# ORNL/HydraGNN

Measured on NVIDIA H100. Metric: atoms_per_sec_training_step, higher is better.
Workload: dtype tf32

## Files before the change

hydragnn_b200/csrc/hgb_painn.cu:

```cuda
#include "hgb_common.cuh"

#define RMAX 8
#define WPB 8

template <int G>
__device__ __forceinline__ float hgb_group_sum(float v, unsigned mask) {
#pragma unroll
  for (int o = G / 2; o > 0; o >>= 1) v += __shfl_xor_sync(mask, v, o);
  return v;
}

#define EPK 12

template <int CPL>
struct ChanVec;
template <>
struct ChanVec<1> {
  static __device__ __forceinline__ void ld(const float* p, float* o) { o[0] = __ldg(p); }
  static __device__ __forceinline__ void st(float* p, const float* o) { p[0] = o[0]; }
};
template <>
struct ChanVec<2> {
  static __device__ __forceinline__ void ld(const float* p, float* o) { const float2 t = __ldg(reinterpret_cast<const float2*>(p)); o[0] = t.x; o[1] = t.y; }
  static __device__ __forceinline__ void st(float* p, const float* o) { *reinterpret_cast<float2*>(p) = make_float2(o[0], o[1]); }
// ... 127 lines not shown
               : "memory");
}

#define TWPB 10
__device__ __forceinline__ float2 pm_lds_f2(uint32_t addr) {
  float2 r;
  asm volatile("ld.shared.v2.f32 {%0, %1}, [%2];" : "=f"(r.x), "=f"(r.y) : "r"(addr));
  return r;
}
__device__ __forceinline__ void pm_cp_async16(void* smem, const void* g) {
  asm volatile("cp.async.ca.shared.global [%0], [%1], 16;" ::"r"((uint32_t)__cvta_generic_to_shared(smem)), "l"(g) : "memory");
}
__device__ __forceinline__ void pm_cp_async_commit() { asm volatile("cp.async.commit_group;" ::: "memory"); }
__device__ __forceinline__ void pm_cp_async_wait_all() { asm volatile("cp.async.wait_group 0;" ::: "memory"); }

template <bool HAS_EF, int RT, int FT>
__global__ void __launch_bounds__(TWPB * 32, 2)
painn_message_fwd_tiled_kernel(const float* __restrict__ phi, const float* __restrict__ s, const float* __restrict__ v,
                               const int32_t* __restrict__ rowptr, const float* __restrict__ rec, const float* __restrict__ wf,
                               const float* __restrict__ bf, const float* __restrict__ efilt, int n, int f_rt, int r, int tn,
                               float* __restrict__ s_out, float* __restrict__ v_out) {
  extern __shared__ __align__(128) uint8_t pm_smem[];
  const int f = FT ? FT : f_rt;
  const int f3 = 3 * f;
  const uint32_t tile_bytes = (uint32_t)tn * f3 * 4;
  auto sphi = [&](int b) { return reinterpret_cast<float*>(pm_smem + (size_t)(2 * b) * tile_bytes); };
  auto sv = [&](int b) { return reinterpret_cast<float*>(pm_smem + (size_t)(2 * b + 1) * tile_bytes); };
  uint64_t* full = reinterpret_cast<uint64_t*>(pm_smem + 4 * (size_t)tile_bytes);
  uint64_t* empty = full + 2;
  float4* scr = reinterpret_cast<float4*>(full + 4) + (threadIdx.x >> 5) * 96;
  const int lane = threadIdx.x & 31, warp = threadIdx.x >> 5;
  const int ntiles = (n + tn - 1) / tn;
  const int ncb = f >> 6;
  if (threadIdx.x == 0) {
    pm_mbar_init(full, 1);
    pm_mbar_init(full + 1, 1);
    pm_mbar_init(empty, TWPB);
    pm_mbar_init(empty + 1, TWPB);
    asm volatile("fence.mbarrier_init.release.cluster;" ::: "memory");
  }
  __syncthreads();
  auto issue = [&](int t, int buf) {
    const int n0 = t * tn;
    const uint32_t bytes = (uint32_t)(min(n, n0 + tn) - n0) * f3 * 4;
    pm_mbar_expect_tx(full + buf, 2 * bytes);
    pm_bulk_g2s(sphi(buf), phi + (int64_t)n0 * f3, bytes, full + buf);
    pm_bulk_g2s(sv(buf), v + (int64_t)n0 * f3, bytes, full + buf);
  };
  if (threadIdx.x == 0 && (int)blockIdx.x < ntiles) issue(blockIdx.x, 0);
  const float4* rec4 = reinterpret_cast<const float4*>(rec);
  auto succ = [&](int i, int& tile, int& cb) {
    int in = i + TWPB;
    if (in < min(n, tile * tn + tn)) return in;
    if (++cb == ncb) { cb = 0; tile += (int)gridDim.x; }
    in = tile * tn + warp;
    return (tile < ntiles && in < min(n, tile * tn + tn)) ? in : -1;
  };
  auto stage = [&](int in, int cbn, int lo_n, int hi_n, float4* dst) {
    if (lane < 4 * min(8, hi_n - lo_n)) pm_cp_async16(dst + lane, rec4 + (int64_t)lo_n * 4 + lane);
// ... 13 lines not shown
  int it = 0;
  for (int t = blockIdx.x; t < ntiles; t += gridDim.x, ++it) {
    const int buf = it & 1;
    const int tnext = t + gridDim.x;
    if (warp == 0 && tnext < ntiles) {
      if (it >= 1) pm_mbar_wait(empty + (buf ^ 1), ((it - 1) >> 1) & 1);
      if (lane == 0) issue(tnext, buf ^ 1);
      __syncwarp();
    }
    pm_mbar_wait(full + buf, (it >> 1) & 1);
    const int n0 = t * tn, n1 = min(n, n0 + tn);
    const float* tv = sv(buf);
    const uint32_t tphi_u = pm_smem_u32(sphi(buf)), tv_u = pm_smem_u32(sv(buf));
    for (int cb = 0; cb < ncb; ++cb) {
      const int cc = cb * 64 + lane * 2;
      float wr[3][2][RT + 1];
#pragma unroll
      for (int a = 0; a < 3; ++a)
#pragma unroll
        for (int tt = 0; tt < 2; ++tt) {
#pragma unroll
          for (int q = 0; q < RT; ++q) wr[a][tt][q] = q < r ? __ldg(wf + (a * f + cc + tt) * r + q) : 0.f;
          wr[a][tt][RT] = __ldg(bf + a * f + cc + tt);
        }
      for (int i = n0 + warp; i < n1; i += TWPB) {
        pm_cp_async_wait_all();
        __syncwarp();
        const float4* cur = scr + sb * 48;
        int inn = -1, lo_nn = 0, hi_nn = 0;
        if (in >= 0) {
// ... 10 lines not shown
            e0 = ep[0]; e1 = ep[1]; e2 = ep[2]; e3 = ep[3];
          } else {
            const float4* ep = rec4 + (int64_t)p * 4;
            e0 = __ldg(ep); e1 = __ldg(ep + 1); e2 = __ldg(ep + 2); e3 = __ldg(ep + 3);
          }
          const float rb[8] = {e0.x, e0.y, e0.z, e0.w, e1.x, e1.y, e1.z, e1.w};
          const float fce = e2.x, d[3] = {e2.y, e2.z, e2.w};
          const int j = __float_as_int(e3.x);
          const int e = __float_as_int(e3.y);
          (void)e;
          float pv[3][2], vv[3][2];
          if (j >= n0 && j < n1) {
            const uint32_t off = (uint32_t)((j - n0) * f3 + cc) * 4u;
#pragma unroll
            for (int a = 0; a < 3; ++a) {
              const float2 x2 = pm_lds_f2(tphi_u + off + a * f * 4), y2 = pm_lds_f2(tv_u + off + a * f * 4);
              pv[a][0] = x2.x; pv[a][1] = x2.y; vv[a][0] = y2.x; vv[a][1] = y2.y;
            }
          } else {
            const float* ph = phi + (int64_t)j * f3 + cc;
            const float* vj = v + (int64_t)j * f3 + cc;
#pragma unroll
            for (int a = 0; a < 3; ++a) { ChanVec<2>::ld(ph + a * f, pv[a]); ChanVec<2>::ld(vj + a * f, vv[a]); }
          }
          float ef[3][2];
          if (HAS_EF) {
#pragma unroll
            for (int a = 0; a < 3; ++a) ChanVec<2>::ld(efilt + (int64_t)e * f3 + a * f + cc, ef[a]);
          }
#pragma unroll
          for (int tt = 0; tt < 2; ++tt) {
            float w[3];
#pragma unroll
            for (int a = 0; a < 3; ++a) {
              float acc = wr[a][tt][RT] * fce;
#pragma unroll
              for (int q = 0; q < RT; ++q) acc = fmaf(wr[a][tt][q], rb[q], acc);
              w[a] = HAS_EF ? acc * ef[a][tt] : acc;
            }
            const float gv = w[0] * pv[0][tt], ge = w[1] * pv[1][tt];
            as[tt] = fmaf(w[2], pv[2][tt], as[tt]);
#pragma unroll
            for (int k = 0; k < 3; ++k) av[k][tt] = fmaf(ge, d[k], fmaf(vv[k][tt], gv, av[k][tt]));
          }
        }
        const float2 own_s = *(reinterpret_cast<const float2*>(cur + 32) + lane);
        float so[2] = {own_s.x + as[0], own_s.y + as[1]}, tmp[2];
        ChanVec<2>::st(s_out + (int64_t)i * f + cc, so);
#pragma unroll
        for (int k = 0; k < 3; ++k) {
          const float2 own = *reinterpret_cast<const float2*>(tv + (size_t)(i - n0) * f3 + k * f + cc);
          tmp[0] = own.x + av[k][0]; tmp[1] = own.y + av[k][1];
          ChanVec<2>::st(v_out + (int64_t)i * f3 + k * f + cc, tmp);
        }
        lo = lo_n; hi = hi_n; sb ^= 1;
        in = inn; lo_n = lo_nn; hi_n = hi_nn;
      }
    }
    __syncwarp();
    if (lane == 0) pm_mbar_arrive(empty + buf);
  }
}

static int painn_group(int f) { int g = 32; if (f < 32) { g = 1; while (g < f) g <<= 1; } return g; }
static int painn_cpl(int f) { return (f >= 64 && f % 2 == 0) ? 2 : 1; }

extern "C" int hgb_painn_message_fwd(const float* phi, const float* s, const float* v, const int32_t* rowptr,
                                     const int32_t* perm, const int32_t* nbr, const float* epack, const float* rec, const float* wf,
                                     const float* bf, const float* efilt, int32_t n, int32_t f, int32_t r, float* s_out, float* v_out,
                                     hgb_stream_t stream) {
  HGB_REQUIRE(n >= 0 && f > 0 && r > 0 && r <= RMAX, "painn_message_fwd: need 0 < num_radial <= %d (got %d)", RMAX, r);
  HGB_REQUIRE(phi && s && v && rowptr && nbr && epack && wf && bf && s_out && v_out, "painn_message_fwd: null pointer");
  if (n == 0) return HGB_OK;
  cudaStream_t st = (cudaStream_t)stream;
  if (rec && f % 64 == 0 && f <= 256 && n >= 256 && (((uintptr_t)phi | (uintptr_t)v | (uintptr_t)s | (uintptr_t)rec) % 16 == 0)) {
    int tn = (int)((110 * 1024 - TWPB * 1536 - 64) / ((size_t)4 * 3 * f * 4));
    tn = (tn / TWPB) * TWPB;
    if (tn > 3 * TWPB) tn = 3 * TWPB;
    if (tn < TWPB) tn = TWPB;
    const size_t smem = (size_t)4 * tn * 3 * f * 4 + 64 + TWPB * 1536;
    static bool attr_done = false;
    if (!attr_done) {
#define SETA(E, R) cudaFuncSetAttribute(painn_message_fwd_tiled_kernel<E, R, 64>, cudaFuncAttributeMaxDynamicSharedMemorySize, 227 * 1024); \
                   cudaFuncSetAttribute(painn_message_fwd_tiled_kernel<E, R, 0>, cudaFuncAttributeMaxDynamicSharedMemorySize, 227 * 1024)
      SETA(false, 5); SETA(false, 8); SETA(true, 5); SETA(true, 8);
#undef SETA
      attr_done = true;
    }
    const int ntiles = (n + tn - 1) / tn;
    const int g1 = ntiles < 2 * HGB_NUM_SMS ? ntiles : 2 * HGB_NUM_SMS;
#define LAUNCH_F(E, R, F) painn_message_fwd_tiled_kernel<E, R, F><<<g1, TWPB * 32, smem, st>>>(phi, s, v, rowptr, rec, wf, bf, efilt, n, f, r, tn, s_out, v_out)
#define LAUNCH_T(E, R) do { if (f == 64) LAUNCH_F(E, R, 64); else LAUNCH_F(E, R, 0); } while (0)
    if (efilt) { if (r <= 5) LAUNCH_T(true, 5); else LAUNCH_T(true, 8); }
    else { if (r <= 5) LAUNCH_T(false, 5); else LAUNCH_T(false, 8); }
#undef LAUNCH_T
#undef LAUNCH_F
    HGB_LAUNCH_CHECK("painn_message_fwd_tiled");
    return HGB_OK;
  }
  const int cpl = painn_cpl(f), group = painn_group(f);
  dim3 grid(hgb_grid_for(n, WPB * (32 / group), HGB_NUM_SMS * 8), (f + group * cpl - 1) / (group * cpl));
#define LAUNCH(C, E, G, R) painn_message_fwd_kernel<C, E, G, R><<<grid, WPB * 32, 0, st>>>(phi, s, v, rowptr, perm, nbr, epack, wf, bf, efilt, n, f, r, s_out, v_out)
#define LAUNCH_R(C, E, G) do { if (r <= 5) LAUNCH(C, E, G, 5); else LAUNCH(C, E, G, 8); } while (0)
#define LAUNCH_G(E)                                                        \
  switch (group) {                                                         \
    case 1: LAUNCH_R(1, E, 1); break;                                      \
    case 2: LAUNCH_R(1, E, 2); break;                                      \
// ... 153 lines not shown
          __syncthreads();
          red[warp * 32 + lane] = gw[a][t][q];
          __syncthreads();
          if (warp == 0 && lane < GROUP) {
            float acc = 0.f;
#pragma unroll
            for (int w8 = 0; w8 < WPB; ++w8)
#pragma unroll
              for (int g = 0; g < NPW; ++g) acc += red[w8 * 32 + lane + GROUP * g];
            if (ok) mypart[(a * f + cc + t) * (r + 1) + (q == RT ? r : q)] = acc;
          }
        }
      }
}

template <bool HAS_EF, bool NEED_EDGE, int RT, int FT>
__global__ void __launch_bounds__(WPB * 32, 2)
painn_message_bwd_tiled_kernel(const float* __restrict__ gs_out, const float* __restrict__ gv_out, const float* __restrict__ phi,
                               const float* __restrict__ v, const int32_t* __restrict__ rowptr, const float* __restrict__ rec,
                               const float* __restrict__ wf, const float* __restrict__ bf, const float* __restrict__ efilt, int n,
                               int f_rt, int r, int tn, float* __restrict__ gphi, float* __restrict__ gv, float* __restrict__ part,
                               float* __restrict__ g_epack, float* __restrict__ g_efilt, int multi_cb) {
  extern __shared__ __align__(128) uint8_t pm_smem[];
  const int f = FT ? FT : f_rt;
  const int f3 = 3 * f;
  const uint32_t gs_bytes = (uint32_t)tn * f * 4, gv_bytes = (uint32_t)tn * f3 * 4;
  auto sgs = [&](int b) { return reinterpret_cast<float*>(pm_smem + (size_t)b * (gs_bytes + gv_bytes)); };
  auto sgv = [&](int b) { return reinterpret_cast<float*>(pm_smem + (size_t)b * (gs_bytes + gv_bytes) + gs_bytes); };
  uint64_t* full = reinterpret_cast<uint64_t*>(pm_smem + 2 * ((size_t)gs_bytes + gv_bytes));
  uint64_t* empty = full + 2;
  float* red = reinterpret_cast<float*>(full + 4);
  float4* scr = reinterpret_cast<float4*>(red + WPB * 32) + (threadIdx.x >> 5) * 256;
  const int lane = threadIdx.x & 31, warp = threadIdx.x >> 5;
  const int ntiles = (n + tn - 1) / tn;
  if (threadIdx.x == 0) {
    pm_mbar_init(full, 1);
    pm_mbar_init(full + 1, 1);
// ... 14 lines not shown
  const int cc = cb * 64 + lane * 2;
  float wr[3][2][RT + 1], gw[3][2][RT + 1];
#pragma unroll
  for (int a = 0; a < 3; ++a)
#pragma unroll
    for (int t = 0; t < 2; ++t) {
#pragma unroll
      for (int q = 0; q < RT; ++q) { wr[a][t][q] = q < r ? wf[(a * f + cc + t) * r + q] : 0.f; gw[a][t][q] = 0.f; }
      wr[a][t][RT] = bf[a * f + cc + t];
      gw[a][t][RT] = 0.f;
    }
  const float4* rec4 = reinterpret_cast<const float4*>(rec);
  auto stage = [&](int jn, int lo_n, int hi_n, float4* dst) {
    if (lane < 4 * min(8, hi_n - lo_n)) pm_cp_async16(dst + lane, rec4 + (int64_t)lo_n * 4 + lane);
    const float* pj = phi + (int64_t)jn * f3 + cb * 64;
    const float* vjp = v + (int64_t)jn * f3 + cb * 64;
    pm_cp_async16(dst + 32 + lane, pj + (lane >> 4) * f + (lane & 15) * 4);
    pm_cp_async16(dst + 80 + lane, vjp + (lane >> 4) * f + (lane & 15) * 4);
    if (lane < 16) {
      pm_cp_async16(dst + 64 + lane, pj + 2 * f + lane * 4);
      pm_cp_async16(dst + 112 + lane, vjp + 2 * f + lane * 4);
    }
  };
  auto succ = [&](int j, int& tile) {
    int jn = j + WPB;
    if (jn < min(n, tile * tn + tn)) return jn;
    tile += (int)gridDim.x;
    jn = tile * tn + warp;
    return (tile < ntiles && jn < min(n, tile * tn + tn)) ? jn : -1;
  };
  int lo = 0, hi = 0, sb = 0, lo_n = 0, hi_n = 0, jn = -1, tile_n = blockIdx.x;
  {
    const int j0 = blockIdx.x * tn + warp;
    if ((int)blockIdx.x < ntiles && j0 < min(n, (int)blockIdx.x * tn + tn)) {
      lo = rowptr[j0]; hi = rowptr[j0 + 1];
      stage(j0, lo, hi, scr);
// ... 15 lines not shown
    const int n0 = tile * tn, n1 = min(n, n0 + tn);
    const float* tgv = sgv(buf);
    const uint32_t tgs_u = pm_smem_u32(sgs(buf)), tgv_u = pm_smem_u32(sgv(buf));
    for (int j = n0 + warp; j < n1; j += WPB) {
      pm_cp_async_wait_all();
      __syncwarp();
      const float4* cur = scr + sb * 128;
      int jnn = -1, lo_nn = 0, hi_nn = 0;
      if (jn >= 0) {
        stage(jn, lo_n, hi_n, scr + (sb ^ 1) * 128);
        jnn = succ(jn, tile_n);
        if (jnn >= 0) { lo_nn = rowptr[jnn]; hi_nn = rowptr[jnn + 1]; }
      }
      pm_cp_async_commit();
      float ph[3][2], vj[3][2], aphi[3][2], agv[3][2];
#pragma unroll
      for (int a = 0; a < 3; ++a) {
        const float2 p2 = *(reinterpret_cast<const float2*>(cur + 32 + a * 16) + lane);
        const float2 v2 = *(reinterpret_cast<const float2*>(cur + 80 + a * 16) + lane);
        ph[a][0] = p2.x; ph[a][1] = p2.y; vj[a][0] = v2.x; vj[a][1] = v2.y;
        aphi[a][0] = aphi[a][1] = 0.f; agv[a][0] = agv[a][1] = 0.f;
      }
      for (int p = lo; p < hi; ++p) {
        float4 e0, e1, e2, e3;
        if (p - lo < 8) {
          const float4* ep = cur + (p - lo) * 4;
          e0 = ep[0]; e1 = ep[1]; e2 = ep[2]; e3 = ep[3];
        } else {
          const float4* ep = rec4 + (int64_t)p * 4;
          e0 = __ldg(ep); e1 = __ldg(ep + 1); e2 = __ldg(ep + 2); e3 = __ldg(ep + 3);
        }
        const float rb[8] = {e0.x, e0.y, e0.z, e0.w, e1.x, e1.y, e1.z, e1.w};
        const float fce = e2.x, d[3] = {e2.y, e2.z, e2.w};
        const int i = __float_as_int(e3.x);
        const int e = __float_as_int(e3.y);
// ... 137 lines not shown
  if (threadIdx.y == 0 && t < cnt) {
    float sum = 0.f;
#pragma unroll
    for (int w8 = 0; w8 < 8; ++w8) sum += red[w8][threadIdx.x];
    const int row = t / (r + 1), q = t % (r + 1);
    if (q == r) gbf[row] = sum; else gwf[row * r + q] = sum;
  }
}

static int painn_bwd_grid(int n, int f) { return hgb_grid_for(n, WPB * (32 / painn_group(f)), HGB_NUM_SMS * (f < 32 ? 2 : 4)); }

extern "C" int64_t hgb_painn_message_bwd_workspace_bytes(int32_t n, int32_t f, int32_t r) {
  return (int64_t)painn_bwd_grid(n, f) * 3 * f * (r + 1) * 4;
}

extern "C" int hgb_painn_message_bwd(const float* gs_out, const float* gv_out, const float* phi, const float* v,
                                     const int32_t* rowptr_src, const int32_t* perm_src, const int32_t* nbr_agg, const float* epack,
                                     const float* rec, const float* wf, const float* bf, const float* efilt, int32_t n, int32_t f, int32_t r,
                                     float* gphi, float* gv, float* gwf, float* gbf, float* g_epack, float* g_efilt, void* workspace,
                                     int64_t workspace_bytes, hgb_stream_t stream) {
  HGB_REQUIRE(n >= 0 && f > 0 && r > 0 && r <= RMAX, "painn_message_bwd: need 0 < num_radial <= %d (got %d)", RMAX, r);
  HGB_REQUIRE(gs_out && gv_out && phi && v && rowptr_src && nbr_agg && epack && wf && bf && gphi && gv && gwf && gbf && workspace,
              "painn_message_bwd: null pointer");
  const bool need_edge = g_epack != nullptr;
  HGB_REQUIRE((efilt != nullptr) == (g_efilt != nullptr), "painn_message_bwd: g_efilt iff efilt");
  HGB_REQUIRE(workspace_bytes >= hgb_painn_message_bwd_workspace_bytes(n, f, r), "painn_message_bwd: workspace too small");
  cudaStream_t st = (cudaStream_t)stream;
  const int f3 = 3 * f;
  if (n == 0) {
    cudaMemsetAsync(gwf, 0, (size_t)f3 * r * 4, st);
    cudaMemsetAsync(gbf, 0, (size_t)f3 * 4, st);
    return HGB_OK;
  }
  float* part = (float*)workspace;
  if (rec && f % 64 == 0 && f <= 256 && n >= 256 && (((uintptr_t)gs_out | (uintptr_t)gv_out | (uintptr_t)phi | (uintptr_t)v | (uintptr_t)rec) % 16 == 0)) {
    const size_t fixed = 32 + WPB * 32 * 4 + WPB * 4096;
    int tn = (int)((110 * 1024 - fixed) / ((size_t)2 * 4 * f * 4));
    tn = (tn / WPB) * WPB;
    if (tn > 32) tn = 32;
    if (tn < WPB) tn = WPB;
    const size_t smem = (size_t)2 * tn * 4 * f * 4 + fixed;
    static bool attr_done = false;
    if (!attr_done) {
#define SETA(E, G, R) cudaFuncSetAttribute(painn_message_bwd_tiled_kernel<E, G, R, 64>, cudaFuncAttributeMaxDynamicSharedMemorySize, 227 * 1024); \
                      cudaFuncSetAttribute(painn_message_bwd_tiled_kernel<E, G, R, 0>, cudaFuncAttributeMaxDynamicSharedMemorySize, 227 * 1024)
      SETA(false, false, 5); SETA(false, true, 5); SETA(true, false, 5); SETA(true, true, 5);
      SETA(false, false, 8); SETA(false, true, 8); SETA(true, false, 8); SETA(true, true, 8);
#undef SETA
      attr_done = true;
    }
    const int ntiles = (n + tn - 1) / tn;
    int gx = painn_bwd_grid(n, f);
    if (gx > ntiles) gx = ntiles;
    if (gx > 2 * HGB_NUM_SMS) gx = 2 * HGB_NUM_SMS;
    const int ncb2 = f / 64;
    dim3 grid2(gx, ncb2);
#define LAUNCH_F(E, G, R, F) painn_message_bwd_tiled_kernel<E, G, R, F><<<grid2, WPB * 32, smem, st>>>(gs_out, gv_out, phi, v, rowptr_src, rec, wf, bf, efilt, n, f, r, tn, gphi, gv, part, g_epack, g_efilt, ncb2 > 1)
#define LAUNCH_T(E, G, R) do { if (f == 64) LAUNCH_F(E, G, R, 64); else LAUNCH_F(E, G, R, 0); } while (0)
#define LAUNCH_TR(E, G) do { if (r <= 5) LAUNCH_T(E, G, 5); else LAUNCH_T(E, G, 8); } while (0)
    if (efilt) { if (need_edge) LAUNCH_TR(true, true); else LAUNCH_TR(true, false); }
    else { if (need_edge) LAUNCH_TR(false, true); else LAUNCH_TR(false, false); }
#undef LAUNCH_TR
#undef LAUNCH_T
    HGB_LAUNCH_CHECK("painn_message_bwd_tiled");
    painn_wgrad_reduce_kernel<<<(f3 * (r + 1) + 31) / 32, dim3(32, 8), 0, st>>>(part, gx, f3, r, gwf, gbf);
    HGB_LAUNCH_CHECK("painn_wgrad_reduce");
    return HGB_OK;
  }
  const int cpl = painn_cpl(f), group = painn_group(f);
  const int ncb = (f + group * cpl - 1) / (group * cpl);
  dim3 grid(painn_bwd_grid(n, f), ncb);
#define LAUNCH(C, E, G, W, R) painn_message_bwd_kernel<C, E, G, W, R><<<grid, WPB * 32, 0, st>>>(gs_out, gv_out, phi, v, rowptr_src, perm_src, nbr_agg, epack, wf, bf, efilt, n, f, r, gphi, gv, part, g_epack, g_efilt, ncb > 1)
#define LAUNCH_R(C, E, G, W) do { if (r <= 5) LAUNCH(C, E, G, W, 5); else LAUNCH(C, E, G, W, 8); } while (0)
// ... 282 lines not shown
```

hydragnn_b200/ops.py:

```python
import torch
from torch.autograd.function import once_differentiable

from . import _lib

ACT_CODES = {None: 0, "none": 0, "relu": 1, "silu": 2, "tanh": 3, "sigmoid": 4, "lrelu": 5, "elu": 6, "selu": 7}
POOL_CODES = {"add": 0, "sum": 0, "mean": 1, "max": 2}


def _stream():
    return torch.cuda.current_stream().cuda_stream


def _p(t):
    return None if t is None else t.data_ptr()


def _chk(t, dtype=torch.float32):
    if t is None:
        return None
    if not t.is_cuda:
        raise RuntimeError("hydragnn_b200 ops need CUDA tensors (no CPU fallback on the hot path)")
    if t.dtype != dtype:
        raise RuntimeError("expected %s, got %s" % (dtype, t.dtype))
    return t if t.is_contiguous() else t.contiguous()
# ... 657 lines not shown
        ctx.save_for_backward(unit, ln)
        ctx.r, ctx.cutoff = num_radial, float(cutoff)
        return epack

    @staticmethod
    @once_differentiable
    def backward(ctx, g_epack):
        unit, ln = ctx.saved_tensors
        e = unit.shape[0]
        g_unit = torch.empty_like(unit)
        g_len = torch.empty_like(ln)
        _lib.call("hgb_painn_edge_embed_bwd", _p(unit), _p(ln), _p(_chk(g_epack)), e, ctx.r, ctx.cutoff, _p(g_unit), _p(g_len), _stream())
        return g_unit, g_len, None, None


class PainnMessageFn(torch.autograd.Function):

    @staticmethod
    def forward(ctx, phi, s, v, epack, wf, bf, efilt, plan, rec_row=None):
        n, f = s.shape
        r = wf.shape[1]
        phi, s, v = _chk(phi), _chk(s), _chk(v)
        s_out, v_out = torch.empty_like(s), torch.empty_like(v)
        agg = plan.by_row
        _lib.call("hgb_painn_message_fwd", _p(phi), _p(s), _p(v), _p(agg.rowptr), _p(agg.perm), _p(plan.nbr("row")), _p(epack),
                  _p(rec_row), _p(_chk(wf)), _p(_chk(bf)), _p(_chk(efilt)), n, f, r, _p(s_out), _p(v_out), _stream())
        ctx.save_for_backward(phi, v, epack, wf, bf, efilt)
        ctx.plan, ctx.use_rec = plan, rec_row is not None
        return s_out, v_out

    @staticmethod
    @once_differentiable
    def backward(ctx, gs_out, gv_out):
        phi, v, epack, wf, bf, efilt = ctx.saved_tensors
        plan = ctx.plan
        n, f = gs_out.shape
        r = wf.shape[1]
        gs_out, gv_out = _chk(gs_out), _chk(gv_out)
        need_edge = ctx.needs_input_grad[3]
        gphi, gv = torch.empty_like(phi), torch.empty_like(v)
        gwf, gbf = torch.empty_like(wf), torch.empty_like(bf)
        cpl = 2 if (f >= 64 and f % 2 == 0) else 1
        multi = f > 32 * cpl
        g_epack = (torch.zeros_like(epack) if multi else torch.empty_like(epack)) if need_edge else None
        g_ef = torch.empty_like(efilt) if efilt is not None else None
        nbytes = _lib.query("hgb_painn_message_bwd_workspace_bytes", n, f, r)
        ws = _ws(nbytes, phi.device)
        src = plan.by_col
        rec_col = None
        if ctx.use_rec:
            cache = plan.__dict__.setdefault("_rec_col", {})
            key = epack.data_ptr()
            if key not in cache:
                cache.clear()
                cache[key] = painn_edge_records(epack, plan, "col")
            rec_col = cache[key]
        _lib.call("hgb_painn_message_bwd", _p(gs_out), _p(gv_out), _p(phi), _p(v), _p(src.rowptr), _p(src.perm), _p(plan.nbr("col")),
                  _p(epack), _p(rec_col), _p(wf), _p(bf), _p(efilt), n, f, r, _p(gphi), _p(gv), _p(gwf), _p(gbf), _p(g_epack), _p(g_ef),
                  _p(ws), nbytes, _stream())
        return gphi, gs_out, gv, g_epack, gwf, gbf, g_ef, None, None


def painn_edge_records(epack, plan, which):
    csr = plan.by_row if which == "row" else plan.by_col
    rec = torch.empty(plan.num_edges, 16, dtype=epack.dtype, device=epack.device)
    _lib.call("hgb_painn_edge_records", _p(epack.detach()), _p(csr.perm), _p(plan.nbr(which)), plan.num_edges, _p(rec), _stream())
    return rec


def raw_linear(x2, w, b, code=0, param=0.0, want_z=False):
    m, k = x2.shape
    n = w.shape[0]
    y = torch.empty(m, n, dtype=x2.dtype, device=x2.device)
    z = torch.empty_like(y) if want_z else None
    _lib.call("hgb_linear_fwd", _p(x2), _p(w), _p(b), m, n, k, x2.stride(0), w.stride(0), code, float(param), _p(y), _p(z), _stream())
# ... 821 lines not shown
```

hydragnn_b200/stacks.py:

```python
import torch
import torch.nn.functional as F
from torch import nn

from . import ops
from .ops import GatherRows, LinearAct, MatMul, SegmentSum


def activation_function_selection(name):
    table = {"relu": nn.ReLU, "selu": nn.SELU, "elu": nn.ELU, "sigmoid": nn.Sigmoid,
             "lrelu_01": lambda: nn.LeakyReLU(0.1), "lrelu_025": lambda: nn.LeakyReLU(0.25),
             "lrelu_05": lambda: nn.LeakyReLU(0.5)}
    if name == "prelu":
        raise ValueError("activation 'prelu' (a learnable slope) is not supported by the b200 engine")
    if name not in table:
        raise ValueError("Unknown activation function: " + str(name))
    return table[name]()


def _act_code(mod):
    if isinstance(mod, nn.ReLU):
        return "relu", 0.0
    if isinstance(mod, nn.SiLU):
        return "silu", 0.0
    if isinstance(mod, nn.Tanh):
# ... 200 lines not shown

class PainnMessage(nn.Module):
    def __init__(self, node_size, num_radial, cutoff, edge_dim=None):
        super().__init__()
        self.node_size, self.num_radial, self.cutoff, self.edge_dim = node_size, num_radial, cutoff, edge_dim
        self.scalar_message_mlp = nn.Sequential(nn.Linear(node_size, node_size), nn.SiLU(),
                                                nn.Linear(node_size, node_size * 3))
        self.filter_layer = nn.Linear(num_radial, node_size * 3)
        if edge_dim is not None:
            self.edge_filter = nn.Sequential(nn.Linear(edge_dim, node_size), nn.SiLU(),
                                             nn.Linear(node_size, node_size * 3))

    def forward(self, s, v, plan, geom, edge_attr=None, higher_order=False):
        f = self.node_size
        if higher_order:
            diff, dist = geom["unit"], geom["len"]
            n = torch.arange(1, self.num_radial + 1, device=dist.device)
            rbf = torch.sin(dist * n * torch.pi / self.cutoff) / dist
            fcut = torch.where(dist < self.cutoff, 0.5 * (torch.cos(torch.pi * dist / self.cutoff) + 1.0),
                               torch.zeros_like(dist))
            w = ops.linear_any_order(rbf, self.filter_layer.weight, self.filter_layer.bias) * fcut
            if edge_attr is not None:
                w = w * run_mlp(self.edge_filter, edge_attr, True)
            phi = run_mlp(self.scalar_message_mlp, s, True)
            fo = w * GatherRows.apply(phi, plan.by_col)
            g_v, g_e, m_s = torch.split(fo, f, dim=1)
            m_v = GatherRows.apply(v, plan.by_col) * g_v.unsqueeze(1) + g_e.unsqueeze(1) * (diff / dist).unsqueeze(-1)
            return s + SegmentSum.apply(m_s, plan.by_row), v + SegmentSum.apply(m_v, plan.by_row)
        phi = run_mlp(self.scalar_message_mlp, s)
        efilt = run_mlp(self.edge_filter, edge_attr) if edge_attr is not None else None
        if "rec_row" not in geom and self.node_size % 64 == 0:
            geom["rec_row"] = ops.painn_edge_records(geom["epack"], plan, "row")
        return ops.PainnMessageFn.apply(phi, s, v, geom["epack"], self.filter_layer.weight, self.filter_layer.bias, efilt, plan,
                                        geom.get("rec_row"))


class PainnUpdate(nn.Module):
    def __init__(self, node_size, last_layer=False):
        super().__init__()
        self.update_U = nn.Linear(node_size, node_size)
        self.update_V = nn.Linear(node_size, node_size)
        self.last_layer = last_layer
        self.update_mlp = nn.Sequential(nn.Linear(node_size * 2, node_size), nn.SiLU(),
                                        nn.Linear(node_size, node_size * (2 if last_layer else 3)))

    def forward(self, s, v, higher_order=False):
        f = v.shape[-1]
        if higher_order:
            uv = ops.linear_any_order(v, self.update_U.weight, self.update_U.bias)
# ... 28 lines not shown
class PainnConv(nn.Module):
    def __init__(self, msg, upd, node_embed_out, vec_embed_out):
        super().__init__()
        self.module_0, self.module_1, self.module_2 = msg, upd, node_embed_out
        if vec_embed_out is not None:
            self.module_3 = vec_embed_out
        self.last = vec_embed_out is None

    def forward(self, inv_node_feat, equiv_node_feat, plan, edge_attr=None, edge_shifts=None, geom=None, higher_order=False):
        s, v = self.module_0(inv_node_feat, equiv_node_feat, plan, geom, edge_attr, higher_order)
        s, v_new = self.module_1(s, v, higher_order)
        s = run_mlp(self.module_2, s, higher_order)
        if self.last:
            return s, v
        lin = self.module_3
        v_new = ops.linear_any_order(v_new, lin.weight, lin.bias) if higher_order else ops.linear_act(v_new, lin.weight, lin.bias)
        return s, v_new


class MLPNode(nn.Module):

    def __init__(self, input_dim, output_dim, hidden_dim_node, activation, num_mlp=1, num_nodes=None):
        super().__init__()
        self.num_nodes, self.output_dim = num_nodes, output_dim
        self.mlp = nn.ModuleList()
        for _ in range(num_mlp):
            dims = [input_dim] + list(hidden_dim_node)
            layers = []
            for d0, d1 in zip(dims[:-1], dims[1:]):
                layers += [nn.Linear(d0, d1), activation]
            layers.append(nn.Linear(dims[-1], output_dim))
            self.mlp.append(nn.Sequential(*layers))
# ... 378 lines not shown
```

include/hgb.h:

```cpp
#ifndef HGB_H
#define HGB_H

#include <stdint.h>

#ifdef __cplusplus
extern "C" {
#endif

typedef void* hgb_stream_t;

#define HGB_OK 0
#define HGB_EINVAL (-1)
#define HGB_ECUDA (-2)
#define HGB_ECAPACITY (-3)

#define HGB_ACT_DERIV 100
#define HGB_ACT_NONE 0
#define HGB_ACT_RELU 1
#define HGB_ACT_SILU 2
#define HGB_ACT_TANH 3
#define HGB_ACT_SIGMOID 4
#define HGB_ACT_LRELU 5
#define HGB_ACT_ELU 6
#define HGB_ACT_SELU 7
// ... 95 lines not shown
int hgb_colsum(const float* x, int32_t m, int32_t n, float* out, void* workspace, hgb_stream_t stream);
int64_t hgb_colsum_workspace_bytes(int32_t m, int32_t n);


int hgb_edge_geom_fwd(const float* pos, const int32_t* row, const int32_t* col, const float* shifts,
                      int64_t e, float eps, float* vec, float* len, float* unit, hgb_stream_t stream);
int hgb_edge_geom_bwd(const float* vec, const float* len, float eps, const float* g_vec_in,
                      const float* g_len, const float* g_unit, int64_t e, float* g_vec,
                      hgb_stream_t stream);
int hgb_painn_edge_embed_fwd(const float* unit, const float* len, int64_t e, int32_t r, float cutoff,
                             float* epack, hgb_stream_t stream);
int hgb_painn_edge_embed_bwd(const float* unit, const float* len, const float* g_epack, int64_t e, int32_t r,
                             float cutoff, float* g_unit, float* g_len, hgb_stream_t stream);


int hgb_painn_message_fwd(const float* phi, const float* s, const float* v, const int32_t* rowptr,
                          const int32_t* perm, const int32_t* nbr, const float* epack, const float* rec,
                          const float* wf, const float* bf, const float* efilt, int32_t n, int32_t f, int32_t r,
                          float* s_out, float* v_out, hgb_stream_t stream);
int hgb_painn_edge_records(const float* epack, const int32_t* perm, const int32_t* nbr, int64_t e, float* rec,
                           hgb_stream_t stream);
int hgb_painn_message_bwd(const float* gs_out, const float* gv_out, const float* phi, const float* v,
                          const int32_t* rowptr_src, const int32_t* perm_src, const int32_t* nbr_agg,
                          const float* epack, const float* rec, const float* wf, const float* bf, const float* efilt, int32_t n,
                          int32_t f, int32_t r, float* gphi, float* gv, float* gwf, float* gbf, float* g_epack,
                          float* g_efilt, void* workspace, int64_t workspace_bytes, hgb_stream_t stream);
int64_t hgb_painn_message_bwd_workspace_bytes(int32_t n, int32_t f, int32_t r);

int hgb_painn_update_pre_fwd(const float* vv, int64_t ld, const float* s, int32_t n, int32_t f, float* mlp_in,
                             hgb_stream_t stream);
int hgb_painn_update_post_fwd(const float* a, const float* uv, const float* vv, int64_t ld, const float* s,
                              const float* v, int32_t n, int32_t f, int32_t last, float* s_out,
                              float* v_out, hgb_stream_t stream);
int hgb_painn_update_post_bwd_a(const float* gs_out, const float* gv_out, const float* uv,
                                const float* vv, int64_t ld, int32_t n, int32_t f, int32_t last, float* ga,
                                hgb_stream_t stream);
int hgb_painn_update_bwd(const float* gs_out, const float* gv_out, const float* g_mlp_in,
                         const float* a, const float* uv, const float* vv, int64_t ld, const float* mlp_in,
                         int32_t n, int32_t f, int32_t last, float* guv, float* gvv, float* gs,
                         float* gv, hgb_stream_t stream);
int hgb_painn_update_tc_fwd(const float* v, const float* s, const float* wuv, const float* buv, int32_t n,
// ... 140 lines not shown
```

Baseline: 41.57 million.

## Fuse rank-1 affine vector projection into PaiNN message kernels as lazy AffineV

When the update layer's vector linear has input width 1, its output is kept as a lazy AffineV (v0, weight, bias) rather than materialized as an n×3×f tensor. The forward and backward message kernels then read the 3-float v0 per node and rebuild v on the fly with an FMA. This cuts global and shared-memory traffic for v, and the smaller shared tiles allow more nodes per tile. The weight and bias gradients are computed separately in Python through a small-k backward, which adds a launch and some code-path complexity.

New measurement: 42.85 million (median of 6 runs). +3.1%, better.

```diff
diff --git a/hydragnn_b200/csrc/hgb_painn.cu b/hydragnn_b200/csrc/hgb_painn.cu
--- a/hydragnn_b200/csrc/hgb_painn.cu
+++ b/hydragnn_b200/csrc/hgb_painn.cu
@@ -165,19 +165,30 @@
 __device__ __forceinline__ void pm_cp_async_commit() { asm volatile("cp.async.commit_group;" ::: "memory"); }
 __device__ __forceinline__ void pm_cp_async_wait_all() { asm volatile("cp.async.wait_group 0;" ::: "memory"); }
 
-template <bool HAS_EF, int RT, int FT>
+__device__ __forceinline__ float pm_lds_f1(uint32_t addr) {
+  float r;
+  asm volatile("ld.shared.f32 %0, [%1];" : "=f"(r) : "r"(addr));
+  return r;
+}
+
+#define AV_TILE_BYTES(tn) ((((uint32_t)(tn) * 12u) + 15u) & ~15u)
+
+template <bool HAS_EF, int RT, int FT, bool AV>
 __global__ void __launch_bounds__(TWPB * 32, 2)
 painn_message_fwd_tiled_kernel(const float* __restrict__ phi, const float* __restrict__ s, const float* __restrict__ v,
+                               const float* __restrict__ v_in, const float* __restrict__ v_w, const float* __restrict__ v_b,
                                const int32_t* __restrict__ rowptr, const float* __restrict__ rec, const float* __restrict__ wf,
                                const float* __restrict__ bf, const float* __restrict__ efilt, int n, int f_rt, int r, int tn,
                                float* __restrict__ s_out, float* __restrict__ v_out) {
+  static_assert(!AV || FT == 64, "affine v: one 64-channel block");
   extern __shared__ __align__(128) uint8_t pm_smem[];
   const int f = FT ? FT : f_rt;
   const int f3 = 3 * f;
   const uint32_t tile_bytes = (uint32_t)tn * f3 * 4;
-  auto sphi = [&](int b) { return reinterpret_cast<float*>(pm_smem + (size_t)(2 * b) * tile_bytes); };
-  auto sv = [&](int b) { return reinterpret_cast<float*>(pm_smem + (size_t)(2 * b + 1) * tile_bytes); };
-  uint64_t* full = reinterpret_cast<uint64_t*>(pm_smem + 4 * (size_t)tile_bytes);
+  const uint32_t vt_bytes = AV ? AV_TILE_BYTES(tn) : tile_bytes;
+  auto sphi = [&](int b) { return reinterpret_cast<float*>(pm_smem + (size_t)b * (tile_bytes + vt_bytes)); };
+  auto sv = [&](int b) { return reinterpret_cast<float*>(pm_smem + (size_t)b * (tile_bytes + vt_bytes) + tile_bytes); };
+  uint64_t* full = reinterpret_cast<uint64_t*>(pm_smem + 2 * ((size_t)tile_bytes + vt_bytes));
   uint64_t* empty = full + 2;
   float4* scr = reinterpret_cast<float4*>(full + 4) + (threadIdx.x >> 5) * 96;
   const int lane = threadIdx.x & 31, warp = threadIdx.x >> 5;
@@ -194,6 +205,14 @@
   auto issue = [&](int t, int buf) {
     const int n0 = t * tn;
     const uint32_t bytes = (uint32_t)(min(n, n0 + tn) - n0) * f3 * 4;
+    if (AV) {
+      const uint32_t vb = (uint32_t)(min(n, n0 + tn) - n0) * 12u, vbulk = vb & ~15u;
+      for (uint32_t q = vbulk / 4; q < vb / 4; ++q) sv(buf)[q] = __ldg(v_in + (int64_t)n0 * 3 + q);
+      pm_mbar_expect_tx(full + buf, bytes + vbulk);
+      pm_bulk_g2s(sphi(buf), phi + (int64_t)n0 * f3, bytes, full + buf);
+      if (vbulk) pm_bulk_g2s(sv(buf), v_in + (int64_t)n0 * 3, vbulk, full + buf);
+      return;
+    }
     pm_mbar_expect_tx(full + buf, 2 * bytes);
     pm_bulk_g2s(sphi(buf), phi + (int64_t)n0 * f3, bytes, full + buf);
     pm_bulk_g2s(sv(buf), v + (int64_t)n0 * f3, bytes, full + buf);
@@ -237,6 +256,8 @@
     const uint32_t tphi_u = pm_smem_u32(sphi(buf)), tv_u = pm_smem_u32(sv(buf));
     for (int cb = 0; cb < ncb; ++cb) {
       const int cc = cb * 64 + lane * 2;
+      float aw[2] = {0.f, 0.f}, ab[2] = {0.f, 0.f};
+      if (AV) { aw[0] = __ldg(v_w + cc); aw[1] = __ldg(v_w + cc + 1); ab[0] = __ldg(v_b + cc); ab[1] = __ldg(v_b + cc + 1); }
       float wr[3][2][RT + 1];
 #pragma unroll
       for (int a = 0; a < 3; ++a)
@@ -277,14 +298,28 @@
             const uint32_t off = (uint32_t)((j - n0) * f3 + cc) * 4u;
 #pragma unroll
             for (int a = 0; a < 3; ++a) {
-              const float2 x2 = pm_lds_f2(tphi_u + off + a * f * 4), y2 = pm_lds_f2(tv_u + off + a * f * 4);
-              pv[a][0] = x2.x; pv[a][1] = x2.y; vv[a][0] = y2.x; vv[a][1] = y2.y;
+              const float2 x2 = pm_lds_f2(tphi_u + off + a * f * 4);
+              pv[a][0] = x2.x; pv[a][1] = x2.y;
+              if (AV) {
+                const float x0 = pm_lds_f1(tv_u + (uint32_t)((j - n0) * 3 + a) * 4u);
+                vv[a][0] = fmaf(x0, aw[0], ab[0]); vv[a][1] = fmaf(x0, aw[1], ab[1]);
+              } else {
+                const float2 y2 = pm_lds_f2(tv_u + off + a * f * 4);
+                vv[a][0] = y2.x; vv[a][1] = y2.y;
+              }
             }
           } else {
             const float* ph = phi + (int64_t)j * f3 + cc;
-            const float* vj = v + (int64_t)j * f3 + cc;
-#pragma unroll
-            for (int a = 0; a < 3; ++a) { ChanVec<2>::ld(ph + a * f, pv[a]); ChanVec<2>::ld(vj + a * f, vv[a]); }
+#pragma unroll
+            for (int a = 0; a < 3; ++a) {
+              ChanVec<2>::ld(ph + a * f, pv[a]);
+              if (AV) {
+                const float x0 = __ldg(v_in + (int64_t)j * 3 + a);
+                vv[a][0] = fmaf(x0, aw[0], ab[0]); vv[a][1] = fmaf(x0, aw[1], ab[1]);
+              } else {
+                ChanVec<2>::ld(v + (int64_t)j * f3 + a * f + cc, vv[a]);
+              }
+            }
           }
           float ef[3][2];
           if (HAS_EF) {
@@ -312,7 +347,13 @@
         ChanVec<2>::st(s_out + (int64_t)i * f + cc, so);
 #pragma unroll
         for (int k = 0; k < 3; ++k) {
-          const float2 own = *reinterpret_cast<const float2*>(tv + (size_t)(i - n0) * f3 + k * f + cc);
+          float2 own;
+          if (AV) {
+            const float x0 = tv[(i - n0) * 3 + k];
+            own = make_float2(fmaf(x0, aw[0], ab[0]), fmaf(x0, aw[1], ab[1]));
+          } else {
+            own = *reinterpret_cast<const float2*>(tv + (size_t)(i - n0) * f3 + k * f + cc);
+          }
           tmp[0] = own.x + av[k][0]; tmp[1] = own.y + av[k][1];
           ChanVec<2>::st(v_out + (int64_t)i * f3 + k * f + cc, tmp);
         }
@@ -328,32 +369,41 @@
 static int painn_group(int f) { int g = 32; if (f < 32) { g = 1; while (g < f) g <<= 1; } return g; }
 static int painn_cpl(int f) { return (f >= 64 && f % 2 == 0) ? 2 : 1; }
 
-extern "C" int hgb_painn_message_fwd(const float* phi, const float* s, const float* v, const int32_t* rowptr,
-                                     const int32_t* perm, const int32_t* nbr, const float* epack, const float* rec, const float* wf,
-                                     const float* bf, const float* efilt, int32_t n, int32_t f, int32_t r, float* s_out, float* v_out,
-                                     hgb_stream_t stream) {
+extern "C" int hgb_painn_message_affine_v_supported(int32_t n, int32_t f) { return (f == 64 && n >= 256) ? 1 : 0; }
+
+extern "C" int hgb_painn_message_fwd(const float* phi, const float* s, const float* v, const float* v_in, const float* v_w,
+                                     const float* v_b, const int32_t* rowptr, const int32_t* perm, const int32_t* nbr,
+                                     const float* epack, const float* rec, const float* wf, const float* bf, const float* efilt,
+                                     int32_t n, int32_t f, int32_t r, float* s_out, float* v_out, hgb_stream_t stream) {
   HGB_REQUIRE(n >= 0 && f > 0 && r > 0 && r <= RMAX, "painn_message_fwd: need 0 < num_radial <= %d (got %d)", RMAX, r);
-  HGB_REQUIRE(phi && s && v && rowptr && nbr && epack && wf && bf && s_out && v_out, "painn_message_fwd: null pointer");
+  const bool av = v_in != nullptr;
+  HGB_REQUIRE(phi && s && (av ? (v_w && v_b && !v) : v != nullptr) && rowptr && nbr && epack && wf && bf && s_out && v_out,
+              "painn_message_fwd: null pointer (or both v and v_in)");
+  HGB_REQUIRE(!av || (hgb_painn_message_affine_v_supported(n, f) && rec &&
+                      (((uintptr_t)phi | (uintptr_t)s | (uintptr_t)rec | (uintptr_t)v_in) % 16 == 0)),
+              "painn_message_fwd: affine v needs f = 64, n >= 256, edge records and 16-byte aligned rows (n=%d f=%d)", n, f);
   if (n == 0) return HGB_OK;
   cudaStream_t st = (cudaStream_t)stream;
   if (rec && f % 64 == 0 && f <= 256 && n >= 256 && (((uintptr_t)phi | (uintptr_t)v | (uintptr_t)s | (uintptr_t)rec) % 16 == 0)) {
-    int tn = (int)((110 * 1024 - TWPB * 1536 - 64) / ((size_t)4 * 3 * f * 4));
-    tn = (tn / TWPB) * TWPB;
-    if (tn > 3 * TWPB) tn = 3 * TWPB;
-    if (tn < TWPB) tn = TWPB;
-    const size_t smem = (size_t)4 * tn * 3 * f * 4 + 64 + TWPB * 1536;
+    const size_t fixed = TWPB * 1536 + 64, row = av ? (size_t)2 * 3 * f * 4 + 2 * 12 : (size_t)4 * 3 * f * 4;
+    const int step = av ? 2 * TWPB : TWPB;
+    int tn = (int)((110 * 1024 - fixed) / row);
+    tn = (tn / step) * step;
+    if (tn < step) tn = step;
+    const size_t smem = av ? (size_t)2 * tn * 3 * f * 4 + 2 * AV_TILE_BYTES(tn) + fixed : (size_t)4 * tn * 3 * f * 4 + fixed;
     static bool attr_done = false;
     if (!attr_done) {
-#define SETA(E, R) cudaFuncSetAttribute(painn_message_fwd_tiled_kernel<E, R, 64>, cudaFuncAttributeMaxDynamicSharedMemorySize, 227 * 1024); \
-                   cudaFuncSetAttribute(painn_message_fwd_tiled_kernel<E, R, 0>, cudaFuncAttributeMaxDynamicSharedMemorySize, 227 * 1024)
+#define SETA(E, R) cudaFuncSetAttribute(painn_message_fwd_tiled_kernel<E, R, 64, false>, cudaFuncAttributeMaxDynamicSharedMemorySize, 227 * 1024); \
+                   cudaFuncSetAttribute(painn_message_fwd_tiled_kernel<E, R, 0, false>, cudaFuncAttributeMaxDynamicSharedMemorySize, 227 * 1024); \
+                   cudaFuncSetAttribute(painn_message_fwd_tiled_kernel<E, R, 64, true>, cudaFuncAttributeMaxDynamicSharedMemorySize, 227 * 1024)
       SETA(false, 5); SETA(false, 8); SETA(true, 5); SETA(true, 8);
 #undef SETA
       attr_done = true;
     }
     const int ntiles = (n + tn - 1) / tn;
     const int g1 = ntiles < 2 * HGB_NUM_SMS ? ntiles : 2 * HGB_NUM_SMS;
-#define LAUNCH_F(E, R, F) painn_message_fwd_tiled_kernel<E, R, F><<<g1, TWPB * 32, smem, st>>>(phi, s, v, rowptr, rec, wf, bf, efilt, n, f, r, tn, s_out, v_out)
-#define LAUNCH_T(E, R) do { if (f == 64) LAUNCH_F(E, R, 64); else LAUNCH_F(E, R, 0); } while (0)
+#define LAUNCH_F(E, R, F, A) painn_message_fwd_tiled_kernel<E, R, F, A><<<g1, TWPB * 32, smem, st>>>(phi, s, v, v_in, v_w, v_b, rowptr, rec, wf, bf, efilt, n, f, r, tn, s_out, v_out)
+#define LAUNCH_T(E, R) do { if (av) LAUNCH_F(E, R, 64, true); else if (f == 64) LAUNCH_F(E, R, 64, false); else LAUNCH_F(E, R, 0, false); } while (0)
     if (efilt) { if (r <= 5) LAUNCH_T(true, 5); else LAUNCH_T(true, 8); }
     else { if (r <= 5) LAUNCH_T(false, 5); else LAUNCH_T(false, 8); }
 #undef LAUNCH_T
@@ -537,13 +587,15 @@
       }
 }
 
-template <bool HAS_EF, bool NEED_EDGE, int RT, int FT>
+template <bool HAS_EF, bool NEED_EDGE, int RT, int FT, bool AV>
 __global__ void __launch_bounds__(WPB * 32, 2)
 painn_message_bwd_tiled_kernel(const float* __restrict__ gs_out, const float* __restrict__ gv_out, const float* __restrict__ phi,
-                               const float* __restrict__ v, const int32_t* __restrict__ rowptr, const float* __restrict__ rec,
+                               const float* __restrict__ v, const float* __restrict__ v_in, const float* __restrict__ v_w,
+                               const float* __restrict__ v_b, const int32_t* __restrict__ rowptr, const float* __restrict__ rec,
                                const float* __restrict__ wf, const float* __restrict__ bf, const float* __restrict__ efilt, int n,
                                int f_rt, int r, int tn, float* __restrict__ gphi, float* __restrict__ gv, float* __restrict__ part,
                                float* __restrict__ g_epack, float* __restrict__ g_efilt, int multi_cb) {
+  static_assert(!AV || FT == 64, "affine v: one 64-channel block");
   extern __shared__ __align__(128) uint8_t pm_smem[];
   const int f = FT ? FT : f_rt;
   const int f3 = 3 * f;
@@ -588,12 +640,16 @@
   auto stage = [&](int jn, int lo_n, int hi_n, float4* dst) {
     if (lane < 4 * min(8, hi_n - lo_n)) pm_cp_async16(dst + lane, rec4 + (int64_t)lo_n * 4 + lane);
     const float* pj = phi + (int64_t)jn * f3 + cb * 64;
-    const float* vjp = v + (int64_t)jn * f3 + cb * 64;
     pm_cp_async16(dst + 32 + lane, pj + (lane >> 4) * f + (lane & 15) * 4);
-    pm_cp_async16(dst + 80 + lane, vjp + (lane >> 4) * f + (lane & 15) * 4);
-    if (lane < 16) {
-      pm_cp_async16(dst + 64 + lane, pj + 2 * f + lane * 4);
-      pm_cp_async16(dst + 112 + lane, vjp + 2 * f + lane * 4);
+    if (lane < 16) pm_cp_async16(dst + 64 + lane, pj + 2 * f + lane * 4);
+    if (AV) {
+      if (lane < 3)
+        asm volatile("cp.async.ca.shared.global [%0], [%1], 4;" ::"r"(pm_smem_u32(reinterpret_cast<float*>(dst + 80) + lane)),
+                     "l"(v_in + (int64_t)jn * 3 + lane) : "memory");
+    } else {
+      const float* vjp = v + (int64_t)jn * f3 + cb * 64;
+      pm_cp_async16(dst + 80 + lane, vjp + (lane >> 4) * f + (lane & 15) * 4);
+      if (lane < 16) pm_cp_async16(dst + 112 + lane, vjp + 2 * f + lane * 4);
     }
   };
   auto succ = [&](int j, int& tile) {
@@ -639,11 +695,19 @@
       }
       pm_cp_async_commit();
       float ph[3][2], vj[3][2], aphi[3][2], agv[3][2];
+      const float* x0 = reinterpret_cast<const float*>(cur + 80);
+      float2 aw = make_float2(0.f, 0.f), ab = aw;
+      if (AV) { aw = make_float2(__ldg(v_w + cc), __ldg(v_w + cc + 1)); ab = make_float2(__ldg(v_b + cc), __ldg(v_b + cc + 1)); }
 #pragma unroll
       for (int a = 0; a < 3; ++a) {
         const float2 p2 = *(reinterpret_cast<const float2*>(cur + 32 + a * 16) + lane);
-        const float2 v2 = *(reinterpret_cast<const float2*>(cur + 80 + a * 16) + lane);
-        ph[a][0] = p2.x; ph[a][1] = p2.y; vj[a][0] = v2.x; vj[a][1] = v2.y;
+        ph[a][0] = p2.x; ph[a][1] = p2.y;
+        if (AV) {
+          vj[a][0] = fmaf(x0[a], aw.x, ab.x); vj[a][1] = fmaf(x0[a], aw.y, ab.y);
+        } else {
+          const float2 v2 = *(reinterpret_cast<const float2*>(cur + 80 + a * 16) + lane);
+          vj[a][0] = v2.x; vj[a][1] = v2.y;
+        }
         aphi[a][0] = aphi[a][1] = 0.f; agv[a][0] = agv[a][1] = 0.f;
       }
       for (int p = lo; p < hi; ++p) {
@@ -811,14 +875,19 @@
   return (int64_t)painn_bwd_grid(n, f) * 3 * f * (r + 1) * 4;
 }
 
-extern "C" int hgb_painn_message_bwd(const float* gs_out, const float* gv_out, const float* phi, const float* v,
-                                     const int32_t* rowptr_src, const int32_t* perm_src, const int32_t* nbr_agg, const float* epack,
-                                     const float* rec, const float* wf, const float* bf, const float* efilt, int32_t n, int32_t f, int32_t r,
-                                     float* gphi, float* gv, float* gwf, float* gbf, float* g_epack, float* g_efilt, void* workspace,
-                                     int64_t workspace_bytes, hgb_stream_t stream) {
+extern "C" int hgb_painn_message_bwd(const float* gs_out, const float* gv_out, const float* phi, const float* v, const float* v_in,
+                                     const float* v_w, const float* v_b, const int32_t* rowptr_src, const int32_t* perm_src,
+                                     const int32_t* nbr_agg, const float* epack, const float* rec, const float* wf, const float* bf,
+                                     const float* efilt, int32_t n, int32_t f, int32_t r, float* gphi, float* gv, float* gwf, float* gbf,
+                                     float* g_epack, float* g_efilt, void* workspace, int64_t workspace_bytes, hgb_stream_t stream) {
   HGB_REQUIRE(n >= 0 && f > 0 && r > 0 && r <= RMAX, "painn_message_bwd: need 0 < num_radial <= %d (got %d)", RMAX, r);
-  HGB_REQUIRE(gs_out && gv_out && phi && v && rowptr_src && nbr_agg && epack && wf && bf && gphi && gv && gwf && gbf && workspace,
-              "painn_message_bwd: null pointer");
+  const bool av = v_in != nullptr;
+  HGB_REQUIRE(gs_out && gv_out && phi && (av ? (v_w && v_b && !v) : v != nullptr) && rowptr_src && nbr_agg && epack && wf && bf &&
+              gphi && gv && gwf && gbf && workspace,
+              "painn_message_bwd: null pointer (or both v and v_in)");
+  HGB_REQUIRE(!av || (hgb_painn_message_affine_v_supported(n, f) && rec &&
+                      (((uintptr_t)gs_out | (uintptr_t)gv_out | (uintptr_t)phi | (uintptr_t)rec) % 16 == 0)),
+              "painn_message_bwd: affine v needs f = 64, n >= 256, edge records and 16-byte aligned rows (n=%d f=%d)", n, f);
   const bool need_edge = g_epack != nullptr;
   HGB_REQUIRE((efilt != nullptr) == (g_efilt != nullptr), "painn_message_bwd: g_efilt iff efilt");
   HGB_REQUIRE(workspace_bytes >= hgb_painn_message_bwd_workspace_bytes(n, f, r), "painn_message_bwd: workspace too small");
@@ -839,8 +908,9 @@
     const size_t smem = (size_t)2 * tn * 4 * f * 4 + fixed;
     static bool attr_done = false;
     if (!attr_done) {
-#define SETA(E, G, R) cudaFuncSetAttribute(painn_message_bwd_tiled_kernel<E, G, R, 64>, cudaFuncAttributeMaxDynamicSharedMemorySize, 227 * 1024); \
-                      cudaFuncSetAttribute(painn_message_bwd_tiled_kernel<E, G, R, 0>, cudaFuncAttributeMaxDynamicSharedMemorySize, 227 * 1024)
+#define SETA(E, G, R) cudaFuncSetAttribute(painn_message_bwd_tiled_kernel<E, G, R, 64, false>, cudaFuncAttributeMaxDynamicSharedMemorySize, 227 * 1024); \
+                      cudaFuncSetAttribute(painn_message_bwd_tiled_kernel<E, G, R, 0, false>, cudaFuncAttributeMaxDynamicSharedMemorySize, 227 * 1024); \
+                      cudaFuncSetAttribute(painn_message_bwd_tiled_kernel<E, G, R, 64, true>, cudaFuncAttributeMaxDynamicSharedMemorySize, 227 * 1024)
       SETA(false, false, 5); SETA(false, true, 5); SETA(true, false, 5); SETA(true, true, 5);
       SETA(false, false, 8); SETA(false, true, 8); SETA(true, false, 8); SETA(true, true, 8);
 #undef SETA
@@ -852,8 +922,8 @@
     if (gx > 2 * HGB_NUM_SMS) gx = 2 * HGB_NUM_SMS;
     const int ncb2 = f / 64;
     dim3 grid2(gx, ncb2);
-#define LAUNCH_F(E, G, R, F) painn_message_bwd_tiled_kernel<E, G, R, F><<<grid2, WPB * 32, smem, st>>>(gs_out, gv_out, phi, v, rowptr_src, rec, wf, bf, efilt, n, f, r, tn, gphi, gv, part, g_epack, g_efilt, ncb2 > 1)
-#define LAUNCH_T(E, G, R) do { if (f == 64) LAUNCH_F(E, G, R, 64); else LAUNCH_F(E, G, R, 0); } while (0)
+#define LAUNCH_F(E, G, R, F, A) painn_message_bwd_tiled_kernel<E, G, R, F, A><<<grid2, WPB * 32, smem, st>>>(gs_out, gv_out, phi, v, v_in, v_w, v_b, rowptr_src, rec, wf, bf, efilt, n, f, r, tn, gphi, gv, part, g_epack, g_efilt, ncb2 > 1)
+#define LAUNCH_T(E, G, R) do { if (av) LAUNCH_F(E, G, R, 64, true); else if (f == 64) LAUNCH_F(E, G, R, 64, false); else LAUNCH_F(E, G, R, 0, false); } while (0)
 #define LAUNCH_TR(E, G) do { if (r <= 5) LAUNCH_T(E, G, 5); else LAUNCH_T(E, G, 8); } while (0)
     if (efilt) { if (need_edge) LAUNCH_TR(true, true); else LAUNCH_TR(true, false); }
     else { if (need_edge) LAUNCH_TR(false, true); else LAUNCH_TR(false, false); }
diff --git a/hydragnn_b200/ops.py b/hydragnn_b200/ops.py
--- a/hydragnn_b200/ops.py
+++ b/hydragnn_b200/ops.py
@@ -1,3 +1,5 @@
+from typing import NamedTuple
+
 import torch
 from torch.autograd.function import once_differentiable
 
@@ -695,31 +697,56 @@
         return g_unit, g_len, None, None
 
 
+class AffineV(NamedTuple):
+    v0: torch.Tensor
+    weight: torch.Tensor
+    bias: torch.Tensor
+
+    def materialize(self, higher_order=False):
+        return linear_any_order(self.v0, self.weight, self.bias) if higher_order else linear_act(self.v0, self.weight, self.bias)
+
+
+def painn_affine_v_ok(v, s, rec_row):
+    n, f = s.shape
+    return (isinstance(v, AffineV) and rec_row is not None and s.is_cuda and v.v0.is_contiguous() and v.v0.data_ptr() % 16 == 0
+            and bool(_lib.query("hgb_painn_message_affine_v_supported", n, f)))
+
+
 class PainnMessageFn(torch.autograd.Function):
 
     @staticmethod
-    def forward(ctx, phi, s, v, epack, wf, bf, efilt, plan, rec_row=None):
+    def forward(ctx, phi, s, v, epack, wf, bf, efilt, plan, rec_row=None, v0=None, vw=None, vb=None):
         n, f = s.shape
         r = wf.shape[1]
-        phi, s, v = _chk(phi), _chk(s), _chk(v)
-        s_out, v_out = torch.empty_like(s), torch.empty_like(v)
+        phi, s = _chk(phi), _chk(s)
+        av = v0 is not None
+        if av:
+            v, v0, vw, vb = None, _chk(v0), _chk(vw), _chk(vb)
+            v_out = torch.empty(n, 3, f, dtype=s.dtype, device=s.device)
+        else:
+            v = _chk(v)
+            v_out = torch.empty_like(v)
+        s_out = torch.empty_like(s)
         agg = plan.by_row
-        _lib.call("hgb_painn_message_fwd", _p(phi), _p(s), _p(v), _p(agg.rowptr), _p(agg.perm), _p(plan.nbr("row")), _p(epack),
-                  _p(rec_row), _p(_chk(wf)), _p(_chk(bf)), _p(_chk(efilt)), n, f, r, _p(s_out), _p(v_out), _stream())
-        ctx.save_for_backward(phi, v, epack, wf, bf, efilt)
+        _lib.call("hgb_painn_message_fwd", _p(phi), _p(s), _p(v), _p(v0), _p(vw), _p(vb), _p(agg.rowptr), _p(agg.perm),
+                  _p(plan.nbr("row")), _p(epack), _p(rec_row), _p(_chk(wf)), _p(_chk(bf)), _p(_chk(efilt)), n, f, r, _p(s_out),
+                  _p(v_out), _stream())
+        ctx.save_for_backward(phi, v, epack, wf, bf, efilt, v0, vw, vb)
         ctx.plan, ctx.use_rec = plan, rec_row is not None
         return s_out, v_out
 
     @staticmethod
     @once_differentiable
     def backward(ctx, gs_out, gv_out):
-        phi, v, epack, wf, bf, efilt = ctx.saved_tensors
+        phi, v, epack, wf, bf, efilt, v0, vw, vb = ctx.saved_tensors
         plan = ctx.plan
         n, f = gs_out.shape
         r = wf.shape[1]
         gs_out, gv_out = _chk(gs_out), _chk(gv_out)
         need_edge = ctx.needs_input_grad[3]
-        gphi, gv = torch.empty_like(phi), torch.empty_like(v)
+        av = v0 is not None
+        gphi = torch.empty_like(phi)
+        gv = torch.empty(n, 3, f, dtype=phi.dtype, device=phi.device)
         gwf, gbf = torch.empty_like(wf), torch.empty_like(bf)
         cpl = 2 if (f >= 64 and f % 2 == 0) else 1
         multi = f > 32 * cpl
@@ -736,10 +763,14 @@
                 cache.clear()
                 cache[key] = painn_edge_records(epack, plan, "col")
             rec_col = cache[key]
-        _lib.call("hgb_painn_message_bwd", _p(gs_out), _p(gv_out), _p(phi), _p(v), _p(src.rowptr), _p(src.perm), _p(plan.nbr("col")),
-                  _p(epack), _p(rec_col), _p(wf), _p(bf), _p(efilt), n, f, r, _p(gphi), _p(gv), _p(gwf), _p(gbf), _p(g_epack), _p(g_ef),
-                  _p(ws), nbytes, _stream())
-        return gphi, gs_out, gv, g_epack, gwf, gbf, g_ef, None, None
+        _lib.call("hgb_painn_message_bwd", _p(gs_out), _p(gv_out), _p(phi), _p(v), _p(v0), _p(vw), _p(vb), _p(src.rowptr),
+                  _p(src.perm), _p(plan.nbr("col")), _p(epack), _p(rec_col), _p(wf), _p(bf), _p(efilt), n, f, r, _p(gphi), _p(gv),
+                  _p(gwf), _p(gbf), _p(g_epack), _p(g_ef), _p(ws), nbytes, _stream())
+        if not av:
+            return gphi, gs_out, gv, g_epack, gwf, gbf, g_ef, None, None, None, None, None
+        g_v0, g_vw, g_vb = raw_smallk_bwd(gv.reshape(3 * n, f), None, None, v0.reshape(3 * n, 1), vw, 0, 0.0,
+                                          ctx.needs_input_grad[9], ctx.needs_input_grad[10], ctx.needs_input_grad[11])
+        return gphi, gs_out, None, g_epack, gwf, gbf, g_ef, None, None, (g_v0.reshape(v0.shape) if g_v0 is not None else None), g_vw, g_vb
 
 
 def painn_edge_records(epack, plan, which):
diff --git a/hydragnn_b200/stacks.py b/hydragnn_b200/stacks.py
--- a/hydragnn_b200/stacks.py
+++ b/hydragnn_b200/stacks.py
@@ -238,6 +238,8 @@
     def forward(self, s, v, plan, geom, edge_attr=None, higher_order=False):
         f = self.node_size
         if higher_order:
+            if isinstance(v, ops.AffineV):
+                v = v.materialize(True)
             diff, dist = geom["unit"], geom["len"]
             n = torch.arange(1, self.num_radial + 1, device=dist.device)
             rbf = torch.sin(dist * n * torch.pi / self.cutoff) / dist
@@ -255,8 +257,12 @@
         efilt = run_mlp(self.edge_filter, edge_attr) if edge_attr is not None else None
         if "rec_row" not in geom and self.node_size % 64 == 0:
             geom["rec_row"] = ops.painn_edge_records(geom["epack"], plan, "row")
-        return ops.PainnMessageFn.apply(phi, s, v, geom["epack"], self.filter_layer.weight, self.filter_layer.bias, efilt, plan,
-                                        geom.get("rec_row"))
+        args = (phi, s, v, geom["epack"], self.filter_layer.weight, self.filter_layer.bias, efilt, plan, geom.get("rec_row"))
+        if isinstance(v, ops.AffineV):
+            if ops.painn_affine_v_ok(v, s, geom.get("rec_row")):
+                return ops.PainnMessageFn.apply(*args[:2], None, *args[3:], *v)
+            args = args[:2] + (v.materialize(),) + args[3:]
+        return ops.PainnMessageFn.apply(*args)
 
 
 class PainnUpdate(nn.Module):
@@ -315,8 +321,11 @@
         if self.last:
             return s, v
         lin = self.module_3
-        v_new = ops.linear_any_order(v_new, lin.weight, lin.bias) if higher_order else ops.linear_act(v_new, lin.weight, lin.bias)
-        return s, v_new
+        if higher_order:
+            return s, ops.linear_any_order(v_new, lin.weight, lin.bias)
+        if lin.in_features == 1 and isinstance(self.module_0, PainnMessage):
+            return s, ops.AffineV(v_new, lin.weight, lin.bias)
+        return s, ops.linear_act(v_new, lin.weight, lin.bias)
 
 
 class MLPNode(nn.Module):
diff --git a/include/hgb.h b/include/hgb.h
--- a/include/hgb.h
+++ b/include/hgb.h
@@ -133,17 +133,19 @@
                              float cutoff, float* g_unit, float* g_len, hgb_stream_t stream);
 
 
-int hgb_painn_message_fwd(const float* phi, const float* s, const float* v, const int32_t* rowptr,
-                          const int32_t* perm, const int32_t* nbr, const float* epack, const float* rec,
-                          const float* wf, const float* bf, const float* efilt, int32_t n, int32_t f, int32_t r,
-                          float* s_out, float* v_out, hgb_stream_t stream);
+int hgb_painn_message_fwd(const float* phi, const float* s, const float* v, const float* v_in, const float* v_w,
+                          const float* v_b, const int32_t* rowptr, const int32_t* perm, const int32_t* nbr,
+                          const float* epack, const float* rec, const float* wf, const float* bf, const float* efilt,
+                          int32_t n, int32_t f, int32_t r, float* s_out, float* v_out, hgb_stream_t stream);
+int hgb_painn_message_affine_v_supported(int32_t n, int32_t f);
 int hgb_painn_edge_records(const float* epack, const int32_t* perm, const int32_t* nbr, int64_t e, float* rec,
                            hgb_stream_t stream);
-int hgb_painn_message_bwd(const float* gs_out, const float* gv_out, const float* phi, const float* v,
-                          const int32_t* rowptr_src, const int32_t* perm_src, const int32_t* nbr_agg,
-                          const float* epack, const float* rec, const float* wf, const float* bf, const float* efilt, int32_t n,
-                          int32_t f, int32_t r, float* gphi, float* gv, float* gwf, float* gbf, float* g_epack,
-                          float* g_efilt, void* workspace, int64_t workspace_bytes, hgb_stream_t stream);
+int hgb_painn_message_bwd(const float* gs_out, const float* gv_out, const float* phi, const float* v, const float* v_in,
+                          const float* v_w, const float* v_b, const int32_t* rowptr_src, const int32_t* perm_src,
+                          const int32_t* nbr_agg, const float* epack, const float* rec, const float* wf, const float* bf,
+                          const float* efilt, int32_t n, int32_t f, int32_t r, float* gphi, float* gv, float* gwf,
+                          float* gbf, float* g_epack, float* g_efilt, void* workspace, int64_t workspace_bytes,
+                          hgb_stream_t stream);
 int64_t hgb_painn_message_bwd_workspace_bytes(int32_t n, int32_t f, int32_t r);
 
 int hgb_painn_update_pre_fwd(const float* vv, int64_t ld, const float* s, int32_t n, int32_t f, float* mlp_in,
```
